# eth-ait/GauSTAR

Measured on AMD Instinct MI355X. Metric: views/sec fwd+bwd @1920x1080, 500k Gaussians; HBM GB/s vs roofline, higher is better.
Workload: dtype f32

## Files before the change

gaustar_amd/csrc/gsr_api.hip:

```cpp
#include "../../include/gsr.h"
#include "gsr_entry.h"
#include "gsr_internal.h"
#include "gsr_plan.h"
#include <algorithm>
#include <cmath>
#include <cstdio>
#include <cstdlib>
#include <cstring>
#include <string>
#include <vector>
#include <atomic>
#include <chrono>
#include <map>
#include <mutex>
#include <utility>

using namespace gsr;

namespace gsr { uint64_t* g_trace = nullptr; }

namespace {
thread_local std::string g_err;
thread_local uint32_t g_pinned_seq = 0;
thread_local uint32_t* g_pinned = nullptr;
// ... 657 lines not shown
int gsr_backward(int P, int D, int M, int R, int num_segments, const float* background, int W, int H,
                 const float* means3D, const float* shs, const float* colors_precomp, const float* scales,
                 float scale_modifier, const float* rotations, const float* cov3D_precomp, const float* viewmatrix,
                 const float* projmatrix, const float* campos, float tan_fovx, float tan_fovy, const int* radii,
                 const void* geom_buffer, const void* binning_buffer, const void* image_buffer, const float* dL_dpix,
                 void* grad_scratch, float* dL_dmean2D, float* dL_dopacity, float* dL_dcolor, float* dL_dmean3D,
                 float* dL_dcov3D, float* dL_dsh, float* dL_dscale, float* dL_drot, gsr_stream_t stream)
{
    return gsr_backward_mt(P, D, M, R, num_segments, 3, background, W, H, means3D, shs, colors_precomp, scales,
                           scale_modifier, rotations, cov3D_precomp, viewmatrix, projmatrix, campos, tan_fovx, tan_fovy,
                           radii, geom_buffer, binning_buffer, image_buffer, dL_dpix, grad_scratch, dL_dmean2D,
                           dL_dopacity, dL_dcolor, dL_dmean3D, dL_dcov3D, dL_dsh, dL_dscale, dL_drot, 0, stream);
}

int gsr_backward_mt(int P, int D, int M, int R, int num_segments, int num_channels, const float* background, int W,
                    int H, const float* means3D,
                 const float* shs, const float* colors_precomp, const float* scales, float scale_modifier,
                 const float* rotations, const float* cov3D_precomp, const float* viewmatrix, const float* projmatrix,
                 const float* campos, float tan_fovx, float tan_fovy, const int* radii, const void* geom_buffer,
                 const void* binning_buffer, const void* image_buffer, const float* dL_dpix, void* grad_scratch,
                 float* dL_dmean2D, float* dL_dopacity, float* dL_dcolor, float* dL_dmean3D, float* dL_dcov3D,
                 float* dL_dsh, float* dL_dscale, float* dL_drot, int grad_scratch_zeroed, gsr_stream_t stream)
{
    g_err.clear();
    if (P <= 0) return 0;
    if (W <= 0 || H <= 0) return fail_msg("gsr_backward: image size must be positive");
    if (!means3D || !viewmatrix || !projmatrix || !campos || !radii || !geom_buffer || !image_buffer || !dL_dpix ||
        !background)
        return fail_msg("gsr_backward: required pointer is null");
    if (!grad_scratch || !dL_dmean2D || !dL_dopacity || !dL_dcolor || !dL_dmean3D || (cov3D_precomp && !dL_dcov3D))
        return fail_msg("gsr_backward: required gradient pointer is null");
    if (shs && !dL_dsh) return fail_msg("gsr_backward: dL_dsh is null in SH mode");
    if (!cov3D_precomp && (!scales || !rotations || !dL_dscale || !dL_drot))
        return fail_msg("gsr_backward: scales/rotations and their gradients are required without cov3D_precomp");
    if (R > 0 && !binning_buffer) return fail_msg("gsr_backward: binning_buffer is null");
    if (R > 0 && num_segments <= 0)
        return fail_msg("gsr_backward: num_segments of the forward is required (a forward-only render cannot be differentiated)");
    if (!channels_ok(num_channels)) return fail_msg("gsr_backward: num_channels must be 3, 4 or 6");
    if (num_channels != 3 && !colors_precomp)
        return fail_msg("gsr_backward: multi-target renders need precomputed colours [P, num_channels]");
    const int C = num_channels;
    hipStream_t st = (hipStream_t)stream;
    ImageState im = carve_image(const_cast<void*>(image_buffer), W, H);
    GeomState g = carve_geom(const_cast<void*>(geom_buffer), P);
    BinState b = carve_bin(const_cast<void*>(binning_buffer), nonneg(R), nonneg(num_segments), C);
    float* grad_acc = static_cast<float*>(grad_scratch);
    if (!grad_scratch_zeroed) {
        Scope sc(ST_ZERO_FILL, st);
        GSR_CHECK(hipMemsetAsync(grad_acc, 0, gsr_grad_scratch_bytes(P), st));
    }
    if (R > 0) {
        {
            Scope sc(ST_BLEND_BWD, st);
            launch_blend_bwd(C, W, H, num_segments, background, features_of(colors_precomp, g), g, im, b, dL_dpix, grad_acc, env_on("GSR_BWD_LIVE"), st);
        }
        GSR_CHECK_LAUNCH("blend_bwd_kernel");
    }
    {
        Scope sc(ST_GEOM_BWD, st);
        const ViewArgs v = view_args(P, D, M, means3D, shs, colors_precomp, nullptr, cov3D_precomp ? nullptr : scales, scale_modifier,
                                     cov3D_precomp ? nullptr : rotations, cov3D_precomp, viewmatrix, projmatrix, campos, W, H,
                                     tan_fovx, tan_fovy, const_cast<int*>(radii));
        launch_geom_bwd(v, g, C, grad_acc, dL_dmean2D, dL_dopacity, dL_dcolor, dL_dmean3D, dL_dcov3D, shs ? dL_dsh : nullptr,
                        cov3D_precomp ? nullptr : dL_dscale, cov3D_precomp ? nullptr : dL_drot, st);
    }
    GSR_CHECK_LAUNCH("geom_bwd_kernel");
    return 0;
}

int gsr_mark_visible(int P, const float* means3D, const float* viewmatrix, const float* projmatrix, uint8_t* present,
                     gsr_stream_t stream)
{
    (void)projmatrix;
    g_err.clear();
    if (P <= 0) return 0;
    if (!means3D || !viewmatrix || !present) return fail_msg("gsr_mark_visible: required pointer is null");
    launch_mark_visible(P, means3D, viewmatrix, present, (hipStream_t)stream);
    GSR_CHECK_LAUNCH("mark_visible_kernel");
    return 0;
}

int gsr_release_stream_state(gsr_stream_t stream)
{
    g_err.clear();
    hipStream_t st = (hipStream_t)stream;
    int dev = 0;
    GSR_CHECK(hipGetDevice(&dev));
    std::lock_guard<std::mutex> lk(g_cnt_mu);
    auto it = g_cnt.find(std::make_pair(dev, st));
    if (it == g_cnt.end()) return 0;
    if (it->second.busy.exchange(true)) return fail_msg("gsr_release_stream_state: a forward on this stream is in flight");
    if (it->second.base) { GSR_CHECK(hipStreamSynchronize(st)); GSR_CHECK(hipFree(it->second.base)); }
    g_cnt.erase(it);
    return 0;
}

namespace {
__global__ void __launch_bounds__(64) camera_key_kernel(const float* __restrict__ m, long long s0, long long s1, uint32_t* __restrict__ pad,
                                                        uint32_t seq)
{
    const int lane = threadIdx.x;
    if (lane < 16) pad[lane] = __float_as_uint(m[(long long)(lane >> 2) * s0 + (long long)(lane & 3) * s1]);
    __threadfence_system();
    if (lane == 0) __hip_atomic_store(&pad[16], seq, __ATOMIC_RELEASE, __HIP_MEMORY_SCOPE_SYSTEM);
}
std::mutex g_key_mu;
std::map<int, hipStream_t> g_key_stream;
// ... 188 lines not shown
```

gaustar_amd/csrc/gsr_blend_bwd.hip:

```cpp
#include "gsr_bwd_util.h"

namespace gsr {

#ifndef GSR_QUAD_WAVES
#define GSR_QUAD_WAVES 7
#endif
#ifndef GSR_QUAD_WAVES4
#define GSR_QUAD_WAVES4 7
#endif
#ifndef GSR_QUAD_WAVES6
#define GSR_QUAD_WAVES6 5
#endif
#ifndef GSR_QUAD_EXP
#define GSR_QUAD_EXP 0
#endif

#ifndef GSR_QUAD_Q
#define GSR_QUAD_Q 32
#endif
#ifndef GSR_QUAD_Q6
#define GSR_QUAD_Q6 32
#endif
template <int C> struct QuadLds {
    static constexpr int Q = C == 6 ? GSR_QUAD_Q6 : GSR_QUAD_Q;
    static_assert(Q == 16 || Q == 32, "whole trips");
    static constexpr int REC_B = C <= 4 ? 48 : 64;
    static constexpr int MOM_B = C <= 4 ? 48 : 64;
    static constexpr int STG_B = C <= 4 ? 32 : 48;
    static constexpr int REC = 0;
    static constexpr int MOM = REC + (Q + 1) * REC_B;
    static constexpr int STG = MOM + (Q + 1) * MOM_B;
    static constexpr int LST = STG + 64 * STG_B;
    static constexpr int ORW = LST + 4 * Q + 16;
    static constexpr int TOTAL = ORW + 32;
    static_assert(STG % 16 == 0 && MOM % 16 == 0 && LST % 16 == 0 && ORW % 16 == 0, "16-byte accesses");
    static_assert((REC_B / 16) * Q < 256 && 6 + C + 2 <= MOM_B / 4, "list bytes; two pad words per moment record");
};

typedef uint32_t u32x2q __attribute__((ext_vector_type(2)));

__device__ __forceinline__ float fold32(float a, float b)
{
    const u32x2q r = __builtin_amdgcn_permlane32_swap(__float_as_uint(a), __float_as_uint(b), false, false);
    return __uint_as_float(r[0]) + __uint_as_float(r[1]);
}
__device__ __forceinline__ float fold16(float a, float b)
{
    const u32x2q r = __builtin_amdgcn_permlane16_swap(__float_as_uint(a), __float_as_uint(b), false, false);
    return __uint_as_float(r[0]) + __uint_as_float(r[1]);
}
__device__ __forceinline__ float fold_quad(float v)
{
    float t = v + __uint_as_float((uint32_t)__builtin_amdgcn_update_dpp(0, (int)__float_as_uint(v), 0xB1, 0xf, 0xf, true));
    return t + __uint_as_float((uint32_t)__builtin_amdgcn_update_dpp(0, (int)__float_as_uint(t), 0x4E, 0xf, 0xf, true));
}

template <int C>
__global__ void __launch_bounds__(64) __attribute__((amdgpu_waves_per_eu(C == 6 ? GSR_QUAD_WAVES6 : C == 4 ? GSR_QUAD_WAVES4 : GSR_QUAD_WAVES, 8)))
blend_bwd_kernel(int W, int H, int gx, const uint4* __restrict__ unit_info, const float4* __restrict__ snap,
                      const uint2* __restrict__ masks, const uint32_t* __restrict__ point_list, const float4* __restrict__ rec_a,
                      const float4* __restrict__ rec_b, const RecTail<C>* __restrict__ rec_c, const float* __restrict__ bg,
                      const float* __restrict__ final_T, const uint32_t* __restrict__ n_contrib,
                      const float* __restrict__ dL_dpix, float* __restrict__ grad_acc, uint64_t* __restrict__ trace,
                      const uint32_t* __restrict__ order, uint32_t live_off)
{
    using L = QuadLds<C>;
    const uint64_t t_start = trace ? wall_clock64() : 0;
    constexpr int Q = L::Q, REC_B = L::REC_B, MOM_B = L::MOM_B, STG_B = L::STG_B, REC = L::REC, MOM = L::MOM, STG = L::STG, LST = L::LST,
                  ORW = L::ORW, TOTAL = L::TOTAL, RV = REC_B / 16;
    static_assert(C == 3 || C == 4 || C == 6, "channel counts of the C ABI");
    constexpr int SV = snap_vecs(C), NM = 6 + C;
    __shared__ __attribute__((aligned(16))) unsigned char lds[TOTAL];
    const uint32_t n_units = gridDim.x >> 2;
    const uint32_t xcd = blockIdx.x & 7u, slot_id = blockIdx.x >> 3;
    const uint32_t grp = slot_id >> 2;
    uint32_t unit = (grp >> 3) * 64u + xcd * 8u + (grp & 7u);
    uint32_t wave_sel = slot_id & 3u;
    const uint32_t full = (n_units >> 6) << 6;
    if (blockIdx.x >= full * 4u) { unit = blockIdx.x >> 2; wave_sel = blockIdx.x & 3u; }
    if (order != nullptr) unit = order[unit];
    const uint4 info = unit_info[unit];
    const uint32_t live4 = (info.x >> UNIT_LIVE_SHIFT) | live_off;
    const int tile = (int)(info.x & UNIT_TILE_MASK);
    const uint32_t list0 = info.y;
    const int n = (int)info.z;
    const uint32_t unit0 = info.w;
    const int s0 = (int)(unit - unit0) * 64;
    if ((s0 >= n) | (((live4 >> wave_sel) & 1u) == 0u)) return;
    const int wave = (int)wave_sel, lane = threadIdx.x;
    const int tx = tile % gx, ty = tile / gx;
    const int sx = tx * TILE + (wave & 1) * SUB, sy = ty * TILE + (wave >> 1) * SUB;
    const int px = sx + (lane & 7), py = sy + (lane >> 3);
    const bool inside = px < W && py < H;
    const int s1 = min(s0 + BSEG, n);
    const bool has_next = s1 < n;
    const uint32_t pix = (uint32_t)W * (uint32_t)py + (uint32_t)px;
    const uint32_t HW = (uint32_t)H * (uint32_t)W;
    const auto at32 = [](const auto* base, uint32_t byte_off) {
        return *reinterpret_cast<std::remove_reference_t<decltype(*base)>*>(reinterpret_cast<const char*>(base) + byte_off);
    };
    float T_final = 0.f;
    int my_last = 0;
    float dp[C];
#pragma unroll
    for (int ch = 0; ch < C; ch++) dp[ch] = 0.f;
    if (inside) {
        T_final = at32(final_T, pix * 4u);
        my_last = (int)at32(n_contrib, pix * 4u);
#pragma unroll
        for (int ch = 0; ch < C; ch++) dp[ch] = at32(dL_dpix, ((uint32_t)ch * HW + pix) * 4u);
    }
    const uint2* const my_words = masks + ((size_t)unit * 4 + wave) * 64 + (uint32_t)lane;
    const uint2* const words_u = masks + ((size_t)unit * 4 + wave) * 64;
    uint2 word = at32(words_u, (uint32_t)lane * 8u);
    uint2 word_next = at32(words_u + (has_next ? 256 : 0), (uint32_t)lane * 8u);
    const int pidx = 16 * (py - ty * TILE) + (px - tx * TILE);
    float Ts, Tf, cs[C], cf[C];
// ... 38 lines not shown
            const uint32_t u_end = unit0 + (uint32_t)(n + 63) / 64u;
            const auto words_of = [&](uint32_t u) { const uint2 w_ = my_words[(size_t)(u - unit) * 256]; return w_.x | w_.y; };
            do { useg++; } while (useg + 1u < u_end && words_of(useg) == 0u);
            load_snapshot<C>(snap + ((size_t)useg * 256 + pidx) * SV, Ts, cs);
        }
        const float inv = __builtin_amdgcn_rcpf(Ts);
        T = Ts;
#pragma unroll
        for (int ch = 0; ch < C; ch++) acc[ch] = (cf[ch] - cs[ch]) * inv;
    }
    float accd = 0.f;
#pragma unroll
    for (int ch = 0; ch < C; ch++) accd = __builtin_fmaf(acc[ch], dp[ch], accd);
    {
        const int lim = my_lim - s0;
        word.x &= lim >= 32 ? 0xffffffffu : lim > 0 ? (1u << lim) - 1u : 0u;
        word.y &= lim >= 64 ? 0xffffffffu : lim > 32 ? (1u << (lim - 32)) - 1u : 0u;
    }
    const uint32_t lds0 = lds_byte_address(lds);
    unsigned long long ks[4];
    {
        const uint32_t sub = (uint32_t)(((lane >> 5) << 1) | ((lane >> 2) & 1));
        const uint32_t ad = lds0 + ORW + 8u * sub;
        const u32x2q zero = {0u, 0u}, mine = {word.x, word.y};
        u32x4 a01, a23;
        asm volatile("ds_write_b64 %2, %3\n\t"
                     "ds_or_b64 %2, %4\n\t"
                     "ds_read_b128 %0, %5\n\t"
                     "ds_read_b128 %1, %5 offset:16\n\t"
                     "s_waitcnt lgkmcnt(0)"
                     : "=&v"(a01), "=&v"(a23) : "v"(ad), "v"(zero), "v"(mine), "v"(lds0 + ORW) : "memory");
        const auto rfl = [](uint32_t v) { return (uint32_t)__builtin_amdgcn_readfirstlane((int)v); };
        ks[0] = ((unsigned long long)rfl(a01[1]) << 32) | rfl(a01[0]);
        ks[1] = ((unsigned long long)rfl(a01[3]) << 32) | rfl(a01[2]);
        ks[2] = ((unsigned long long)rfl(a23[1]) << 32) | rfl(a23[0]);
        ks[3] = ((unsigned long long)rfl(a23[3]) << 32) | rfl(a23[2]);
    }
    const unsigned long long kany = ks[0] | ks[1] | ks[2] | ks[3];
    if (kany == 0ull) return;
    {
        float4* st = reinterpret_cast<float4*>(lds + STG + STG_B * lane);
        st[0] = make_float4(T, accd, __uint_as_float((uint32_t)my_lim), tf_bg);
        st[1] = make_float4(dp[0], dp[1], dp[2], C > 3 ? dp[3 < C ? 3 : 0] : 0.f);
        if constexpr (C == 6) st[2] = make_float4(dp[4 < C ? 4 : 0], dp[5 < C ? 5 : 0], 0.f, 0.f);
    }
    const bool keep = ((kany >> (63 - lane)) & 1ull) != 0ull;
    const unsigned long long m = __ballot(keep);
    const int cnt_all = __popcll(m);
    float4 ra_ = ra, rb_ = rb;
    float rcc[4];
#pragma unroll
    for (int i = 0; i < 4; i++) rcc[i] = i < C - 2 ? rc.c[i < C - 2 ? i : 0] : 0.f;
    uint32_t gid_ = gid;
    for (int q0 = 0; q0 < (GSR_QUAD_EXP == 2 ? 0 : cnt_all); q0 += Q) {
        const int cnt = min(cnt_all - q0, Q);
        const int slot = (int)__builtin_amdgcn_mbcnt_hi((uint32_t)(m >> 32), __builtin_amdgcn_mbcnt_lo((uint32_t)m, 0u)) - q0;
        const bool mine = ((m >> lane) & 1ull) != 0ull && slot >= 0 && slot < Q;
        if (q0 > 0) {
            const uint32_t kl2 = (uint32_t)(min(s0 + 63 - lane, n - 1) - s0);
            ra_ = at32(rec_a + list0 + s0, kl2 * 16u);
            rb_ = at32(rec_b + list0 + s0, kl2 * 16u);
            const RecTail<C> rc2 = at32(rec_c + list0 + s0, kl2 * (uint32_t)sizeof(RecTail<C>));
#pragma unroll
            for (int i = 0; i < C - 2; i++) rcc[i] = rc2.c[i];
            gid_ = at32(point_list + list0 + s0, kl2 * 4u);
        }
        if (mine) {
            float4* r = reinterpret_cast<float4*>(lds + REC + slot * REC_B);
            r[0] = make_float4(ra_.x, ra_.y, ra_.z, ra_.w);
            r[1] = make_float4(rb_.x, rb_.y, __uint_as_float((uint32_t)(s0 + 63 - lane)), __uint_as_float(gid_));
            r[2] = make_float4(rb_.z, rb_.w, rcc[0], rcc[1]);
            if constexpr (C == 6) r[3] = make_float4(rcc[2], rcc[3], 0.f, 0.f);
        }
        if (lane == 0) {
            float4* r = reinterpret_cast<float4*>(lds + REC + Q * REC_B);
            r[0] = make_float4(0.f, 0.f, 0.f, 0.f);
            r[1] = make_float4(0.f, 0.f, __uint_as_float(0x7fffffffu), 0.f);
            r[2] = make_float4(0.f, 0.f, 0.f, 0.f);
            if constexpr (C == 6) r[3] = make_float4(0.f, 0.f, 0.f, 0.f);
        }
        for (int i = lane; i < (Q + 1) * (MOM_B / 16); i += 64) reinterpret_cast<float4*>(lds + MOM)[i] = make_float4(0.f, 0.f, 0.f, 0.f);
        if (lane < Q + 4) reinterpret_cast<uint32_t*>(lds + LST)[lane] = 0x01010101u * (uint32_t)(RV * Q);
        __builtin_amdgcn_wave_barrier();
        int cnt_s[4];
#pragma unroll
        for (int s = 0; s < 4; s++) {
            const bool in_s = mine && ((ks[s] >> (63 - lane)) & 1ull) != 0ull;
            const unsigned long long ms = __ballot(in_s);
            cnt_s[s] = __popcll(ms);
            if (in_s) {
                const int rank = (int)__builtin_amdgcn_mbcnt_hi((uint32_t)(ms >> 32), __builtin_amdgcn_mbcnt_lo((uint32_t)ms, 0u));
                lds[LST + s * Q + (rank & 3) * (Q / 4) + (rank >> 2)] = (unsigned char)(RV * slot);
            }
        }
        __builtin_amdgcn_wave_barrier();
#pragma unroll 1
        for (int s = 0; s < (GSR_QUAD_EXP ? 0 : 4); s++) {
            const int ns = s == 0 ? cnt_s[0] : s == 1 ? cnt_s[1] : s == 2 ? cnt_s[2] : cnt_s[3];
            if (ns == 0) continue;
            int lane_o = lane;
            if constexpr (C == 4) asm volatile("" : "+v"(lane_o));
            const int rho = lane_o >> 4, jj = (lane_o >> 2) & 3, kap = lane_o & 3;
            const int mom_idx = kap == 0 ? ((rho & 1) * 2 + (rho >> 1))
                              : kap == 1 ? 4 + ((rho & 1) * 2 + (rho >> 1))
                              : (kap == 2 && C == 6) ? 8 + ((rho & 1) * 2 + (rho >> 1))
                              : (kap == 2 && rho == 0) ? 8
                              : (kap == 2 && rho == 2 && C == 4) ? 9
                                                                 : NM + (lane_o & 1);
            const int bx = s & 1, by = s >> 1;
            const int pl = 8 * (4 * by + rho) + 4 * bx + kap;
            const float4* st = reinterpret_cast<const float4*>(lds + STG + STG_B * pl);
            const float4 s_a = st[0], s_b = st[1];
            float d4 = 0.f, d5 = 0.f;
            if constexpr (C == 6) { const float4 s_c = st[2]; d4 = s_c.x; d5 = s_c.y; }
            float Tp = s_a.x, Ap = s_a.y;
            const int lim = (int)__float_as_uint(s_a.z);
            const float tfbg = s_a.w;
            const float d0 = s_b.x, d1 = s_b.y, d2 = s_b.z, d3 = s_b.w;
            const float pxf = (float)(sx + 4 * bx + kap), pyf = (float)(sy + 4 * by + rho);
            const int ntrip = (ns + 3) >> 2;
            SlotRegs<RV> rec;
            const uint32_t lst_ad = lds0 + LST + (uint32_t)(s * Q + jj * (Q / 4));
            uint32_t idx_nxt;
            asm volatile("ds_read_u8 %0, %1\n\ts_waitcnt lgkmcnt(0)" : "=v"(idx_nxt) : "v"(lst_ad) : "memory");
            uint32_t ad = (idx_nxt << 4) + (lds0 + REC);
            lds_request<RV, 0>(rec, ad);
            asm volatile("ds_read_u8 %0, %1 offset:1" : "=v"(idx_nxt) : "v"(lst_ad) : "memory");
#pragma unroll 1
            for (int t = 0; t < ntrip; t++) {
                lds_wait<0>(rec);
                asm volatile("" : "+v"(idx_nxt));
                const uint32_t mom_ad = ad + (uint32_t)(MOM - REC) + 4u * (uint32_t)mom_idx;
                float mom_old;
                asm volatile("ds_read_b32 %0, %1" : "=v"(mom_old) : "v"(mom_ad) : "memory");
// ... 20 lines not shown
                asm volatile("s_nop 1\n\t"
                             "v_mul_f32_dpp %0, %4, %0 row_ror:4 row_mask:0xf bank_mask:0x1\n\t"
                             "v_fmac_f32_dpp %2, %5, %1 row_ror:4 row_mask:0xf bank_mask:0x1\n\t"
                             "s_nop 0\n\t"
                             "v_mul_f32_dpp %0, %0, %0 row_shr:4 row_mask:0xf bank_mask:0xf\n\t"
                             "v_fmac_f32_dpp %2, %2, %1 row_shr:4 row_mask:0xf bank_mask:0xf\n\t"
                             "v_mul_f32_dpp %1, %1, %1 row_shr:4 row_mask:0xf bank_mask:0xf\n\t"
                             "v_mul_f32_dpp %0, %0, %0 row_shr:8 row_mask:0xf bank_mask:0xf\n\t"
                             "s_nop 0\n\t"
                             "v_fmac_f32_dpp %2, %2, %1 row_shr:8 row_mask:0xf bank_mask:0xf\n\t"
                             "v_subrev_f32_dpp %3, %5, %6 row_ror:4 row_mask:0xf bank_mask:0xf\n\t"
                             "s_nop 0\n\t"
                             "v_subrev_f32_dpp %3, %2, %6 row_shr:4 row_mask:0xf bank_mask:0xf"
                             : "+v"(x), "+v"(A), "+v"(B), "=&v"(sdl) : "v"(Tp), "v"(Ap), "v"(kd));
                Tp = x;
                Ap = B;
                const float w = ae * x;
                const float u = __builtin_fmaf(sdl, x, -(rinv * tfbg));
                const float r = live ? G * u : 0.0f;
                typedef float f32x2p __attribute__((ext_vector_type(2)));
                const f32x2p dxy = {dx, dy}, d01 = {d0, d1};
                const f32x2p p12 = r * dxy;
                const f32x2p p34 = p12[0] * dxy;
                const float p5 = p12[1] * dy;
                const f32x2p p67 = w * d01;
                const float p8 = w * d2;
                float p8b = C > 3 ? w * d3 : p8;
                if constexpr (C == 3) asm volatile("" : "+v"(p8b));
                const float f01 = fold32(r, p12[0]), f23 = fold32(p12[1], p34[0]), f45 = fold32(p34[1], p5), f67 = fold32(p67[0], p67[1]),
                            f88 = fold32(p8, p8b);
                float f88b = f88;
                if constexpr (C == 6) f88b = fold32(w * d4, w * d5);
                else asm volatile("" : "+v"(f88b));
                const float gA = fold16(f01, f23);
                const float gB = fold16(f45, f67);
                const float gC = fold16(f88, f88b);
                const float hA = fold_quad(gA), hB = fold_quad(gB), hC = fold_quad(gC);
                const float val = kap == 0 ? hA : kap == 1 ? hB : hC;
                if constexpr (RV == 3) asm volatile("s_waitcnt lgkmcnt(4)" : "+v"(mom_old) : : "memory");
                else asm volatile("s_waitcnt lgkmcnt(5)" : "+v"(mom_old) : : "memory");
                const float mom_new = mom_old + val;
                asm volatile("ds_write_b32 %0, %1" : : "v"(mom_ad), "v"(mom_new) : "memory");
            }
            lds_wait<0>(rec);
            asm volatile("" : "+v"(idx_nxt));
            if (jj == 3) {
                float2* stw = reinterpret_cast<float2*>(lds + STG + STG_B * pl);
                *stw = make_float2(Tp, Ap);
            }
            __builtin_amdgcn_wave_barrier();
        }
        asm volatile("s_waitcnt lgkmcnt(0)" : : : "memory");
        __builtin_amdgcn_wave_barrier();
        for (int idx = lane; idx < cnt * NM; idx += 64) {
            const int e = idx / NM, v = idx - e * NM;
            const size_t g = __float_as_uint(reinterpret_cast<const float*>(lds + REC + e * REC_B)[7]);
            atomic_add_f32(grad_acc + g * GRAD_RS + v, reinterpret_cast<const float*>(lds + MOM + e * MOM_B)[v]);
        }
        __builtin_amdgcn_wave_barrier();
    }
    if (trace && lane == 0) {
        if (wave == 0) trace[2 * unit] = t_start;
        atomicMax((unsigned long long*)&trace[2 * unit + 1], (unsigned long long)wall_clock64());
    }
}

#ifdef GSR_BWD_VARIANT
bool launch_blend_bwd_variant(int C, int W, int H, int U, const float* bg, ImageState im, BinState b, const float* dL_dpix, float* grad_acc,
                              hipStream_t st);
#endif
const uint32_t* g_bwd_order = nullptr;

void launch_blend_bwd(int C, int W, int H, int U, const float* bg, const float* feats, GeomState g, ImageState im,
                      BinState b, const float* dL_dpix, float* grad_acc, bool use_live, hipStream_t st)
{
    (void)feats; (void)g;
    if (U <= 0) return;
    const uint32_t live_off = use_live ? 0u : 0xfu;
#ifdef GSR_BWD_VARIANT
    if (launch_blend_bwd_variant(C, W, H, U, bg, im, b, dL_dpix, grad_acc, st)) return;
#endif
    static const int pad = getenv("GSR_BWD_LDS_PAD") ? atoi(getenv("GSR_BWD_LDS_PAD")) : 0;
    const Tiles t = tiles_of(W, H);
    uint64_t* tr = g_trace ? g_trace + 2 * (size_t)t.T : nullptr;
    if (C == 3)
        blend_bwd_kernel<3><<<4 * U, 64, pad, st>>>(W, H, t.gx, b.unit_info, b.snap, b.masks, b.point_list, b.rec_a, b.rec_b,
                                                    static_cast<const RecTail<3>*>(b.rec_c), bg, im.final_T, im.n_contrib, dL_dpix, grad_acc, tr, g_bwd_order, live_off);
    else if (C == 4)
        blend_bwd_kernel<4><<<4 * U, 64, pad, st>>>(W, H, t.gx, b.unit_info, b.snap, b.masks, b.point_list, b.rec_a, b.rec_b,
                                                    static_cast<const RecTail<4>*>(b.rec_c), bg, im.final_T, im.n_contrib, dL_dpix, grad_acc, tr, g_bwd_order, live_off);
    else
        blend_bwd_kernel<6><<<4 * U, 64, pad, st>>>(W, H, t.gx, b.unit_info, b.snap, b.masks, b.point_list, b.rec_a, b.rec_b,
                                                    static_cast<const RecTail<6>*>(b.rec_c), bg, im.final_T, im.n_contrib, dL_dpix, grad_acc, tr, g_bwd_order, live_off);
}

}
```

gaustar_amd/csrc/gsr_blend_fwd.hip:

```cpp
#include "gsr_internal.h"
#include "gsr_mask.h"
#include "gsr_sort.h"
#include "gsr_plan.h"
#include <cstdlib>

namespace gsr {

#ifndef GSR_FWD_LIGHT_TILES
#define GSR_FWD_LIGHT_TILES 16
#endif
constexpr int FWD_LIGHT_TILES = GSR_FWD_LIGHT_TILES;
static_assert(FWD_LIGHT_TILES >= 1 && FWD_LIGHT_TILES <= 64, "a wave's lanes hold the group's tiles");

template <int C, int CH, int MODE, bool PLANNED = false>
__global__ void __launch_bounds__(256)
blend_fwd_kernel(int W, int H, int gx, const uint2* __restrict__ ranges, const uint32_t* __restrict__ order,
                 uint32_t* point_list, const uint64_t* __restrict__ sort_keys, const float4* __restrict__ g0,
                 const float4* __restrict__ g1,
                 const float* __restrict__ feats, const float* __restrict__ bg, float* __restrict__ out_color,
                 float* __restrict__ final_T, uint32_t* __restrict__ n_contrib, const uint32_t* __restrict__ seg_off,
                 uint2* __restrict__ masks, uint4* __restrict__ unit_info, float4* __restrict__ snap, float4* __restrict__ rec_a, float4* __restrict__ rec_b,
                 RecTail<C>* __restrict__ rec_c, const uint2* __restrict__ part_list, const uint32_t* __restrict__ totals,
                 float4* __restrict__ part_fin, uint32_t* __restrict__ part_last, uint32_t* __restrict__ part_ticket,
                 uint32_t part_grid, bool parts_sort, uint32_t split_n, bool keep,
// ... 158 lines not shown
#endif
#ifndef GSR_FWD_SORT_STAGGER
#define GSR_FWD_SORT_STAGGER 1
#endif
#ifndef GSR_FWD_TAIL_PRIO
#define GSR_FWD_TAIL_PRIO 704
#endif
    const auto prio_by_length = [&]() {
        if (GSR_FWD_TAIL_PRIO && tile_block >= (uint32_t)GSR_FWD_TAIL_PRIO && n > 0u) { __builtin_amdgcn_s_setprio(3); return; }
        if (n > 1024u) __builtin_amdgcn_s_setprio(3);
        else if (n > 704u) __builtin_amdgcn_s_setprio(2);
        else if (n > 448u) __builtin_amdgcn_s_setprio(1);
    };
#if GSR_FWD_SORT_STAGGER
    if (GSR_FWD_TAIL_PRIO && tile_block >= (uint32_t)GSR_FWD_TAIL_PRIO && n > 0u) __builtin_amdgcn_s_setprio(3);
    else switch ((tile_block >> 8) & 3u) {
        case 0: __builtin_amdgcn_s_setprio(3); break;
        case 1: __builtin_amdgcn_s_setprio(2); break;
        case 2: __builtin_amdgcn_s_setprio(1); break;
        default: __builtin_amdgcn_s_setprio(0); break;
    }
#else
    prio_by_length();
#endif
    const uint64_t* ids_lds = nullptr;
    if (!is_part) {
        if (sort_keys != nullptr) {
#ifdef GSR_FWD_PHASES
            if (n >= 1u && n <= 2048u) ids_lds = sort_small_tile(reinterpret_cast<uint64_t*>(smem), sort_keys + list0, point_list + list0, n, [&]() { FWD_PHASE(); });
#else
            if (n >= 1u && n <= 2048u) ids_lds = sort_small_tile(reinterpret_cast<uint64_t*>(smem), sort_keys + list0, point_list + list0, n);
#endif
            __syncthreads();
            FWD_PHASE();
        }
#if GSR_FWD_SORT_STAGGER
        prio_by_length();
#endif
    } else if (parts_sort && sort_keys != nullptr && n <= SORT_SMALL_CAP) {
        sort_small_tile(reinterpret_cast<uint64_t*>(smem), sort_keys + list0, point_list + list0, n);
        __syncthreads();
    }
    const uint32_t* list = point_list + list0;
    const TransposeConsts tc(lane);

    float T = 1.0f;
    float Cc[C];
#pragma unroll
    for (int ch = 0; ch < C; ch++) Cc[ch] = 0.f;
    uint32_t last = 0;
    uint32_t live = 0;
    bool done = !inside;
    uint32_t seg_cur = (is_part && part_c0 != 0u) ? 0xffffffffu : 0u;

    uint32_t gid_nxt[PT];
    float4 a_nxt[PT], b_nxt[PT];
    float col_nxt[PT][C];
    const auto fetch_ids = [&](uint32_t c0) {
#pragma unroll
        for (int q = 0; q < PT; q++) {
            const uint32_t k = c0 + q * 256 + threadIdx.x;
            gid_nxt[q] = k < n ? (ids_lds != nullptr ? (uint32_t)ids_lds[k] : list[k]) : 0xffffffffu;
        }
    };
    const auto fetch_records = [&]() {
#pragma unroll
        for (int q = 0; q < PT; q++) {
            const uint32_t gid = gid_nxt[q];
            a_nxt[q] = make_float4(0.f, 0.f, 1.f, 0.f);
            b_nxt[q] = make_float4(1.f, 0.f, -1.f, 0.f);
#pragma unroll
            for (int ch = 0; ch < C; ch++) col_nxt[q][ch] = 0.f;
            if (gid != 0xffffffffu) {
                a_nxt[q] = g0[gid];
                b_nxt[q] = g1[gid];
                if constexpr (C % 2 == 0) {
                    const float2* pf = reinterpret_cast<const float2*>(feats + (size_t)C * gid);
#pragma unroll
                    for (int ch = 0; ch < C; ch += 2) { const float2 v = pf[ch / 2]; col_nxt[q][ch] = v.x; col_nxt[q][ch + 1] = v.y; }
                } else {
#pragma unroll
                    for (int ch = 0; ch < C; ch++) col_nxt[q][ch] = feats[(size_t)C * gid + ch];
                }
            }
        }
    };
    const auto park = [&](uint32_t c0, bool words_known, bool words_out, bool recs_out) {
        const uint32_t u_lo = c0 >> 6;
#pragma unroll
        for (int q = 0; q < PT; q++) {
            const InstRec<C> rec = make_rec<C>(a_nxt[q], b_nxt[q], col_nxt[q]);
            ga[q * 256 + threadIdx.x] = rec.a;
            gb[q * 256 + threadIdx.x] = rec.b;
            gc[q * 256 + threadIdx.x] = rec.t;
            if (recs_out) {
                const uint32_t k = c0 + q * 256 + threadIdx.x;
                if (k < n) {
                    rec_a[list0 + k] = rec.a;
                    rec_b[list0 + k] = rec.b;
                    rec_c[list0 + k] = rec.t;
                }
            }
            if (c0 + q * 256 + wave * 64 < n) {
                const int hw = 2 * (4 * q + wave);
                uint2* const gm = masks + ((size_t)(unit0 + u_lo + 4 * q + wave) * 4) * 64 + lane;
                if (words_known) {
// ... 5 lines not shown
                    }
                } else {
                    unit_masks(a_nxt[q], b_nxt[q], tx * TILE, ty * TILE, tc, [&](int blk, uint32_t lo, uint32_t hi) {
                        mk[blk][hw][lane] = lo;
                        mk[blk][hw + 1][lane] = hi;
                        if (words_out) gm[blk * 64] = make_uint2(lo, hi);
                    });
                }
            }
        }
    };
    const auto nonempty_words = [&](uint32_t c0) {
        uint32_t nz = 0;
#pragma unroll
        for (int hh = 0; hh < NH; hh++)
            if (c0 + 32u * hh < n) nz |= (mk[wave][hh][lane] != 0u ? 1u : 0u) << hh;
        return nz;
    };
#ifndef GSR_FWD_PIPE
#define GSR_FWD_PIPE 1
#endif
#if GSR_FWD_PIPE
    typedef float f32x4_ __attribute__((ext_vector_type(4)));
    typedef float f32x2_ __attribute__((ext_vector_type(2)));
    using TailRegs = std::conditional_t<sizeof(RecTail<C>) == 4, float, std::conditional_t<sizeof(RecTail<C>) == 8, f32x2_, f32x4_>>;
    struct RecRegs { f32x4_ a, b; TailRegs k; };
    const uint32_t ga_addr = (uint32_t)(size_t)ga, gc_addr = (uint32_t)(size_t)gc;
    const auto request = [&](RecRegs& r, uint32_t slot) {
        const uint32_t ad = ga_addr + slot * 16u;
        asm volatile("ds_read_b128 %0, %1" : "=&v"(r.a) : "v"(ad) : "memory");
        asm volatile("ds_read_b128 %0, %1 offset:%2" : "=&v"(r.b) : "v"(ad), "n"(16 * CH) : "memory");
        const uint32_t ak = gc_addr + slot * (uint32_t)sizeof(RecTail<C>);
        if constexpr (sizeof(RecTail<C>) == 4) asm volatile("ds_read_b32 %0, %1" : "=&v"(r.k) : "v"(ak) : "memory");
        else if constexpr (sizeof(RecTail<C>) == 8) asm volatile("ds_read_b64 %0, %1" : "=&v"(r.k) : "v"(ak) : "memory");
        else asm volatile("ds_read_b128 %0, %1" : "=&v"(r.k) : "v"(ak) : "memory");
    };
    const auto walk = [&](uint32_t c0, uint32_t nz) {
        const uint32_t mk_lane = (uint32_t)(size_t)&mk[wave][0][lane];
        uint32_t cur = 0, nw = 0;
        int h = 0, nh = 0;
        bool stopped = false;
        if (nz != 0u) { h = __builtin_ctz(nz); cur = mk[wave][h][lane]; nz &= nz - 1u; }
        if (nz != 0u) { nh = __builtin_ctz(nz); nw = mk[wave][nh][lane]; nz &= nz - 1u; }
        uint32_t slot = (uint32_t)(h * 32 + __builtin_ctz(cur | 0x80000000u));
        RecRegs rec0, rec1;
        request(rec0, slot);
        asm volatile("s_waitcnt lgkmcnt(0)" : "+v"(rec0.a), "+v"(rec0.b), "+v"(rec0.k) : : "memory");
        const auto trip = [&](RecRegs& rec, RecRegs& nxt) {
            const bool act = cur != 0u;
            if (snaps || is_part) {
                const uint32_t seg_new = (c0 + (uint32_t)h * 32u) / (uint32_t)SNAP_SEG;
                if (act && seg_new != seg_cur) {
                    seg_cur = seg_new;
                    store_snapshot<C>(snap + ((size_t)(unit0 + seg_new * (SNAP_SEG / 64)) * 256 + pix_in_tile) * SV, T, Cc);
                }
            }
            const uint32_t rest = cur & (cur - 1u);
            const bool exhausted = rest == 0u;
            const uint32_t ncur = exhausted ? nw : rest;
            const int nh2 = exhausted ? nh : h;
            const uint32_t nslot = (uint32_t)(nh2 * 32 + __builtin_ctz(ncur | 0x80000000u));
            const int t = __builtin_ctz(nz | 0x80000000u) & (NH - 1);
            uint32_t wnext;
            asm volatile("ds_read_b32 %0, %1" : "=v"(wnext) : "v"(mk_lane + (uint32_t)t * 256u) : "memory");
            request(nxt, nslot);
            asm volatile("" : "+v"(rec.a), "+v"(rec.b), "+v"(rec.k));
            float col[C];
            col[0] = rec.b[2]; col[1] = rec.b[3];
            if constexpr (C == 3) col[2] = rec.k;
            else {
#pragma unroll
                for (int ch = 2; ch < C; ch++) col[ch] = rec.k[ch - 2];
            }
            const float dx = rec.a[0] - pxf, dy = rec.a[1] - pyf;
            const float power = pair_exp2_arg(rec.a[2], rec.a[3], rec.b[0], dx, dy);
            const float alpha = fminf(ALPHA_MAX, rec.b[1] * __builtin_amdgcn_exp2f(power));
            const bool ok = act && power <= 0.0f && alpha >= ALPHA_MIN;
            const float test_T = T * (1.0f - alpha);
            const bool stop = ok && test_T < T_EPS;
            const bool upd = ok != stop;
            const float w = upd ? alpha * T : 0.0f;
#pragma unroll
            for (int ch = 0; ch < C; ch++) Cc[ch] += col[ch] * w;
            T = upd ? test_T : T;
            last = upd ? c0 + slot + 1u : last;
            live |= (upd ? 1u : 0u) << (((c0 + slot) >> 6) & 31u);
            if constexpr (C == 3)
                asm volatile("s_waitcnt lgkmcnt(0)" : "+v"(wnext), "+v"(nxt.a), "+v"(nxt.b), "+v"(nxt.k), "+v"(T), "+v"(last), "+v"(Cc[0]), "+v"(Cc[1]), "+v"(Cc[2]) : : "memory");
            else if constexpr (C == 4)
                asm volatile("s_waitcnt lgkmcnt(0)" : "+v"(wnext), "+v"(nxt.a), "+v"(nxt.b), "+v"(nxt.k), "+v"(T), "+v"(last), "+v"(Cc[0]), "+v"(Cc[1]), "+v"(Cc[2]), "+v"(Cc[3]) : : "memory");
            else
                asm volatile("s_waitcnt lgkmcnt(0)" : "+v"(wnext), "+v"(nxt.a), "+v"(nxt.b), "+v"(nxt.k), "+v"(T), "+v"(last), "+v"(Cc[0]), "+v"(Cc[1]), "+v"(Cc[2]), "+v"(Cc[3]), "+v"(Cc[4]), "+v"(Cc[5]) : : "memory");
            cur = ncur;
            h = nh2;
            nw = exhausted ? (nz != 0u ? wnext : 0u) : nw;
            nh = exhausted ? t : nh;
            nz = exhausted ? (nz & (nz - 1u)) : nz;
            stopped = stopped || stop;
            cur = stop ? 0u : cur;
            nw = stop ? 0u : nw;
            nz = stop ? 0u : nz;
            slot = nslot;
        };
        while (__ballot(cur != 0u) != 0ull) {
            trip(rec0, rec1);
            trip(rec1, rec0);
        }
// ... 363 lines not shown
```

gaustar_amd/csrc/gsr_internal.h:

```cpp
#pragma once
#include <cstdlib>
#include <hip/hip_runtime.h>
#include <stdint.h>
#include <stddef.h>

namespace gsr {

constexpr int TILE = 16;
constexpr int SUB = 8;
constexpr float NEAR_Z = 0.2f;
constexpr float ALPHA_MIN = 1.0f / 255.0f;
constexpr float ALPHA_MAX = 0.99f;
constexpr float T_EPS = 0.0001f;

struct Tiles { int gx, gy, T; };
__host__ __device__ inline Tiles tiles_of(int W, int H)
{
    Tiles t; t.gx = (W + TILE - 1) / TILE; t.gy = (H + TILE - 1) / TILE; t.T = t.gx * t.gy; return t;
}

__host__ __device__ inline size_t align_up(size_t x) { return (x + 255) & ~(size_t)255; }

struct GeomState {
    float4* g0;
// ... 191 lines not shown
    uint32_t n_light;
};

extern uint64_t* g_trace;
extern const uint32_t* g_bwd_order;

struct Camera {
    float view[16];
    float proj[16];
    float campos[3];
    float tan_fovx, tan_fovy, focal_x, focal_y;
    int W, H;
};

struct ViewArgs {
    int P, D, M;
    const float* means3D;
    const float* shs;
    const float* colors_precomp;
    const float* opacities;
    const float* scales;
    float scale_modifier;
    const float* rotations;
    const float* cov3D_precomp;
    const float* viewmatrix;
    const float* projmatrix;
    const float* campos;
    int W, H;
    float tan_fovx, tan_fovy;
    int* radii;
    Tiles tiles() const { return tiles_of(W, H); }
};

void launch_preprocess(const ViewArgs& v, GeomState g, ImageState im, uint32_t view_token, hipStream_t st);
void launch_preprocess_planned(const ViewArgs& v, GeomState g, ImageState im, PlanRun plan, hipStream_t st);
void launch_tile_scan(ImageState im, int T, uint32_t* host_totals, uint32_t host_seq, uint32_t view_token, hipStream_t st);
void launch_scatter(int P, int W, int H, int R, uint32_t max_count, GeomState g, ImageState im, BinState b, hipStream_t st);
void launch_scatter_early(int P, int W, int H, int C, GeomState g, ImageState im, void* binning_base, size_t capacity, hipStream_t st);
bool launch_tile_sort(int W, int H, int R, int U, uint32_t max_count, ImageState im, BinState b, bool blend_sorts_small, hipStream_t st);
bool tile_sort_launches(int R, uint32_t max_count, bool blend_sorts_small);
inline int front_of_order(int R, int T)
{
    const long long bound = ((long long)(R > 0 ? R : 0) / 2017 + 1 + 255) / 256 * 256;
    return (int)(bound < (long long)T ? bound : (long long)T);
}
struct PlanJob;
void launch_blend_fwd_planned(int C, int W, int H, const float* bg, const float* feats, GeomState g, ImageState im, BinState b,
                              float* out_color, bool keep_masks, void* zero_ptr, size_t zero_bytes, PlanRun plan, hipStream_t st,
                              const PlanJob* job = nullptr);
void launch_blend_fwd(int C, int W, int H, int R, int U, uint32_t max_count, const float* bg, const float* feats, GeomState g, ImageState im,
                      BinState b, float* out_color, bool keep_masks, void* zero_ptr, size_t zero_bytes, uint32_t* counters,
                      bool sort_small, hipStream_t st, const PlanJob* job = nullptr, bool* job_rides = nullptr, int num_parts = -1);
void launch_blend_bwd(int C, int W, int H, int U, const float* bg, const float* feats, GeomState g, ImageState im, BinState b,
                      const float* dL_dpix, float* grad_acc, bool use_live, hipStream_t st);
void launch_geom_bwd(const ViewArgs& v, GeomState g, int C, const float* grad_acc, float* dL_dmean2D, float* dL_dopacity,
                     float* dL_dcolor, float* dL_dmean3D, float* dL_dcov3D, float* dL_dsh, float* dL_dscale, float* dL_drot,
                     hipStream_t st);
void launch_mark_visible(int P, const float* means3D, const float* view, uint8_t* present, hipStream_t st);
void preprocess_occupancy(int* exact, int* planned);

#ifdef __HIPCC__
__device__ constexpr float kSH0 = 0.28209479177387814f;
__device__ constexpr float kSH1 = 0.4886025119029199f;
__device__ constexpr float kSH2[5] = {1.0925484305920792f, -1.0925484305920792f, 0.31539156525252005f,
                                      -1.0925484305920792f, 0.5462742152960396f};
__device__ constexpr float kSH3[7] = {-0.5900435899266435f, 2.890611442640554f, -0.4570457994644658f,
                                      0.3731763325901154f, -0.4570457994644658f, 1.445305721320277f,
                                      -0.5900435899266435f};
__device__ constexpr float kSH4[9] = {2.5033429417967046f, -1.7701307697799304f, 0.9461746957575601f,
                                      -0.6690465435572892f, 0.10578554691520431f, -0.6690465435572892f,
                                      0.47308734787878004f, -1.7701307697799304f, 0.6258357354491761f};
constexpr int SH_MAX_BASIS = 25;

struct Vec3 { float x, y, z; };

__device__ __forceinline__ Vec3 load3(const float* p, size_t i) { return Vec3{p[3 * i], p[3 * i + 1], p[3 * i + 2]}; }

__device__ __forceinline__ Vec3 xform43(const Vec3 p, const float* m)
{
    return Vec3{m[0] * p.x + m[4] * p.y + m[8] * p.z + m[12], m[1] * p.x + m[5] * p.y + m[9] * p.z + m[13],
                m[2] * p.x + m[6] * p.y + m[10] * p.z + m[14]};
}
__device__ __forceinline__ float xform4w(const Vec3 p, const float* m)
{
    return m[3] * p.x + m[7] * p.y + m[11] * p.z + m[15];
}

__device__ __forceinline__ float view_depth(const Vec3 p, const float* m)
{
#pragma clang fp contract(off)
    const float yz = m[6] * p.y;
    const float zz = m[10] * p.z;
    return (__builtin_fmaf(m[2], p.x, yz) + zz) + m[14];
}

__device__ __forceinline__ void quat_R(const float4 q, float R[3][3])
{
    const float r = q.x, x = q.y, y = q.z, z = q.w;
    R[0][0] = 1.f - 2.f * (y * y + z * z); R[0][1] = 2.f * (x * y - r * z); R[0][2] = 2.f * (x * z + r * y);
    R[1][0] = 2.f * (x * y + r * z); R[1][1] = 1.f - 2.f * (x * x + z * z); R[1][2] = 2.f * (y * z - r * x);
    R[2][0] = 2.f * (x * z - r * y); R[2][1] = 2.f * (y * z + r * x); R[2][2] = 1.f - 2.f * (x * x + y * y);
}

__device__ __forceinline__ void cov3d_from_scale_rot(const Vec3 s_in, float mod, const float4 q, float c[6])
{
    float R[3][3];
    quat_R(q, R);
// ... 393 lines not shown
```

gaustar_amd/csrc/gsr_sort.h:

```cpp
#pragma once
#include "gsr_internal.h"

namespace gsr {

template <int D>
__device__ __forceinline__ uint32_t lane_xor_u32(uint32_t v)
{
    if constexpr (D == 1) return (uint32_t)__builtin_amdgcn_mov_dpp((int)v, 0xB1, 0xf, 0xf, true);
    else if constexpr (D == 2) return (uint32_t)__builtin_amdgcn_mov_dpp((int)v, 0x4E, 0xf, 0xf, true);
    else if constexpr (D == 4) return (uint32_t)__builtin_amdgcn_ds_swizzle((int)v, 0x101F);
    else if constexpr (D == 8) return (uint32_t)__builtin_amdgcn_ds_swizzle((int)v, 0x201F);
    else if constexpr (D == 16) return (uint32_t)__builtin_amdgcn_ds_swizzle((int)v, 0x401F);
    else return (uint32_t)__shfl_xor((int)v, 32, 64);
}
template <int E, int D>
__device__ __forceinline__ void cross_lane_stage(uint64_t (&v)[E], uint32_t e0, uint32_t k, int lane)
{
    const bool lower = (lane & D) == 0;
#pragma unroll
    for (int r = 0; r < E; r++) {
        const uint64_t pv = ((uint64_t)lane_xor_u32<D>((uint32_t)(v[r] >> 32)) << 32) | lane_xor_u32<D>((uint32_t)v[r]);
        const bool asc = ((e0 + r) & k) == 0;
        const bool take_min = lower == asc;
        const bool gt = v[r] > pv;
// ... 117 lines not shown
#define GSR_SORT_KARY 4
#endif
#if GSR_SORT_KARY == 4
            while (lo < hi) {
                const uint32_t span = hi - lo;
                const uint32_t m1 = lo + (span >> 2), m2 = lo + (span >> 1), m3 = lo + ((3u * span) >> 2);
                const uint64_t a1 = a[m1], b1 = b[d - 1u - m1], a2 = a[m2], b2 = b[d - 1u - m2], a3 = a[m3], b3 = b[d - 1u - m3];
                const bool p1 = a1 < b1, p2 = a2 < b2, p3 = a3 < b3;
                if (!p1) hi = m1;
                else if (!p2) { lo = m1 + 1u; hi = m2; }
                else if (!p3) { lo = m2 + 1u; hi = m3; }
                else lo = m3 + 1u;
            }
#else
            while (lo < hi) {
                const uint32_t mid = (lo + hi) >> 1;
                if (a[mid] < b[d - 1u - mid]) lo = mid + 1u; else hi = mid;
            }
#endif
            const uint32_t ai = lo, bi = d - lo;
            uint64_t ka[E], kb[E];
#pragma unroll
            for (int e = 0; e < E; e++) {
                ka[e] = ai + (uint32_t)e < la ? a[ai + e] : ~0ull;
                kb[e] = bi + (uint32_t)e < lb ? b[bi + e] : ~0ull;
            }
#pragma unroll
            for (int e = 0; e < E; e++) res[e] = ka[e] < kb[E - 1 - e] ? ka[e] : kb[E - 1 - e];
#pragma unroll
            for (int j = E / 2; j > 0; j >>= 1) {
#pragma unroll
                for (int e = 0; e < E; e++) {
                    if ((e & j) == 0) {
                        const uint64_t x = res[e], y = res[e | j];
                        const bool gt = x > y;
                        res[e] = gt ? y : x;
                        res[e | j] = gt ? x : y;
                    }
                }
            }
#pragma unroll
            for (int e = 0; e < E; e++)
                if (o0 + (uint32_t)e < n) B[o0 + e] = res[e];
        }
        __syncthreads();
        stamp();
        uint64_t* t = A; A = B; B = t;
    }
    if (out_keys != nullptr) { for (uint32_t i = tid; i < n; i += 256u) out_keys[i] = A[i]; }
    else { for (uint32_t i = tid; i < n; i += 256u) out[i] = (uint32_t)A[i]; }
    return A;
}

template <class STAMP = NoStamp>
__device__ __forceinline__ const uint64_t* sort_small_tile(uint64_t* __restrict__ s, const uint64_t* __restrict__ gk,
                                                           uint32_t* __restrict__ out, uint32_t n, STAMP stamp = STAMP())
{
    if (n == 1) {
        if (threadIdx.x == 0) out[0] = (uint32_t)gk[0];
        return nullptr;
    }
    if (n <= 512u) return sort_tile_merge<2>(s, gk, out, n, nullptr, stamp);
    if (n <= 1024u) return sort_tile_merge<4>(s, gk, out, n, nullptr, stamp);
    return sort_tile_merge<8>(s, gk, out, n, nullptr, stamp);
}

}
```

Baseline: 5316.

## Cheapen blend-backward flush addressing, hoist sentinel, trim LDS zeroing, 32-bit snapshot offsets

The backward blend flush now uses a multiply-shift in place of integer division and stores a precomputed byte offset (gid times row stride) in the record, so the atomic address is a 32-bit add unless the gradient buffer exceeds 4 GiB. The sentinel record write moves out of the per-batch loop, and moment zeroing covers only cnt records instead of Q+1. The forward snapshot store uses 32-bit byte offsets when the list is small enough. The sort tile selection is also rewritten around configurable E macros whose defaults give the same behaviour. These changes cut integer ALU and LDS work in hot loops, at the cost of added specialised paths and one more kernel argument.

After: 5304. About the same (-0.2%).

```diff
diff --git a/gaustar_amd/csrc/gsr_api.hip b/gaustar_amd/csrc/gsr_api.hip
--- a/gaustar_amd/csrc/gsr_api.hip
+++ b/gaustar_amd/csrc/gsr_api.hip
@@ -733,7 +733,7 @@
     if (R > 0) {
         {
             Scope sc(ST_BLEND_BWD, st);
-            launch_blend_bwd(C, W, H, num_segments, background, features_of(colors_precomp, g), g, im, b, dL_dpix, grad_acc, env_on("GSR_BWD_LIVE"), st);
+            launch_blend_bwd(C, W, H, num_segments, background, features_of(colors_precomp, g), g, im, b, dL_dpix, grad_acc, P, env_on("GSR_BWD_LIVE"), st);
         }
         GSR_CHECK_LAUNCH("blend_bwd_kernel");
     }
diff --git a/gaustar_amd/csrc/gsr_blend_bwd.hip b/gaustar_amd/csrc/gsr_blend_bwd.hip
--- a/gaustar_amd/csrc/gsr_blend_bwd.hip
+++ b/gaustar_amd/csrc/gsr_blend_bwd.hip
@@ -37,6 +37,17 @@
     static_assert((REC_B / 16) * Q < 256 && 6 + C + 2 <= MOM_B / 4, "list bytes; two pad words per moment record");
 };
 
+template <int NM> struct FlushDiv {
+    static_assert(NM == 9 || NM == 10 || NM == 12, "6 + C moments");
+    static constexpr uint32_t MUL = NM == 9 ? 57u : NM == 10 ? 205u : 171u, SHIFT = NM == 9 ? 9u : 11u;
+    static constexpr bool exact_below(uint32_t n)
+    {
+        for (uint32_t i = 0; i < n; i++)
+            if (((i * MUL) >> SHIFT) != i / (uint32_t)NM) return false;
+        return true;
+    }
+};
+
 typedef uint32_t u32x2q __attribute__((ext_vector_type(2)));
 
 __device__ __forceinline__ float fold32(float a, float b)
@@ -62,7 +73,7 @@
                       const float4* __restrict__ rec_b, const RecTail<C>* __restrict__ rec_c, const float* __restrict__ bg,
                       const float* __restrict__ final_T, const uint32_t* __restrict__ n_contrib,
                       const float* __restrict__ dL_dpix, float* __restrict__ grad_acc, uint64_t* __restrict__ trace,
-                      const uint32_t* __restrict__ order, uint32_t live_off)
+                      const uint32_t* __restrict__ order, uint32_t live_off, uint32_t wide_acc)
 {
     using L = QuadLds<C>;
     const uint64_t t_start = trace ? wall_clock64() : 0;
@@ -207,6 +218,14 @@
 #pragma unroll
     for (int i = 0; i < 4; i++) rcc[i] = i < C - 2 ? rc.c[i < C - 2 ? i : 0] : 0.f;
     uint32_t gid_ = gid;
+    if (lane == 0) {
+        float4* r = reinterpret_cast<float4*>(lds + REC + Q * REC_B);
+        r[0] = make_float4(0.f, 0.f, 0.f, 0.f);
+        r[1] = make_float4(0.f, 0.f, __uint_as_float(0x7fffffffu), 0.f);
+        r[2] = make_float4(0.f, 0.f, 0.f, 0.f);
+        if constexpr (C == 6) r[3] = make_float4(0.f, 0.f, 0.f, 0.f);
+    }
+    const uint32_t row_scale = wide_acc ? 1u : (uint32_t)(GRAD_RS * sizeof(float));
     for (int q0 = 0; q0 < (GSR_QUAD_EXP == 2 ? 0 : cnt_all); q0 += Q) {
         const int cnt = min(cnt_all - q0, Q);
         const int slot = (int)__builtin_amdgcn_mbcnt_hi((uint32_t)(m >> 32), __builtin_amdgcn_mbcnt_lo((uint32_t)m, 0u)) - q0;
@@ -223,18 +242,11 @@
         if (mine) {
             float4* r = reinterpret_cast<float4*>(lds + REC + slot * REC_B);
             r[0] = make_float4(ra_.x, ra_.y, ra_.z, ra_.w);
-            r[1] = make_float4(rb_.x, rb_.y, __uint_as_float((uint32_t)(s0 + 63 - lane)), __uint_as_float(gid_));
+            r[1] = make_float4(rb_.x, rb_.y, __uint_as_float((uint32_t)(s0 + 63 - lane)), __uint_as_float(gid_ * row_scale));
             r[2] = make_float4(rb_.z, rb_.w, rcc[0], rcc[1]);
             if constexpr (C == 6) r[3] = make_float4(rcc[2], rcc[3], 0.f, 0.f);
         }
-        if (lane == 0) {
-            float4* r = reinterpret_cast<float4*>(lds + REC + Q * REC_B);
-            r[0] = make_float4(0.f, 0.f, 0.f, 0.f);
-            r[1] = make_float4(0.f, 0.f, __uint_as_float(0x7fffffffu), 0.f);
-            r[2] = make_float4(0.f, 0.f, 0.f, 0.f);
-            if constexpr (C == 6) r[3] = make_float4(0.f, 0.f, 0.f, 0.f);
-        }
-        for (int i = lane; i < (Q + 1) * (MOM_B / 16); i += 64) reinterpret_cast<float4*>(lds + MOM)[i] = make_float4(0.f, 0.f, 0.f, 0.f);
+        for (int i = lane; i < cnt * (MOM_B / 16); i += 64) reinterpret_cast<float4*>(lds + MOM)[i] = make_float4(0.f, 0.f, 0.f, 0.f);
         if (lane < Q + 4) reinterpret_cast<uint32_t*>(lds + LST)[lane] = 0x01010101u * (uint32_t)(RV * Q);
         __builtin_amdgcn_wave_barrier();
         int cnt_s[4];
@@ -361,10 +373,25 @@
         }
         asm volatile("s_waitcnt lgkmcnt(0)" : : : "memory");
         __builtin_amdgcn_wave_barrier();
-        for (int idx = lane; idx < cnt * NM; idx += 64) {
-            const int e = idx / NM, v = idx - e * NM;
-            const size_t g = __float_as_uint(reinterpret_cast<const float*>(lds + REC + e * REC_B)[7]);
-            atomic_add_f32(grad_acc + g * GRAD_RS + v, reinterpret_cast<const float*>(lds + MOM + e * MOM_B)[v]);
+        {
+            static_assert(REC_B == MOM_B, "one byte offset for an instance's record and its moments");
+            static_assert(FlushDiv<NM>::exact_below(Q * NM) && 4u * Q * NM * FlushDiv<NM>::MUL < (1u << 24), "the flush's division");
+            const uint32_t end4 = (uint32_t)(cnt * NM) * 4u;
+            const auto flush = [&](auto wide) {
+                for (uint32_t i4 = (uint32_t)lane * 4u; i4 < end4; i4 += 256u) {
+                    const uint32_t e = __umul24(i4, FlushDiv<NM>::MUL) >> (FlushDiv<NM>::SHIFT + 2);
+                    const uint32_t eo = __umul24(e, (uint32_t)MOM_B);
+                    const uint32_t v4 = i4 - __umul24(e, 4u * NM);
+                    const uint32_t row = *reinterpret_cast<const uint32_t*>(lds + REC + 28 + eo);
+                    const float sum = *reinterpret_cast<const float*>(lds + MOM + (i4 + __umul24(e, (uint32_t)(MOM_B - 4 * NM))));
+                    if constexpr (!decltype(wide)::value)
+                        atomic_add_f32(reinterpret_cast<float*>(reinterpret_cast<char*>(grad_acc) + (row + v4)), sum);
+                    else
+                        atomic_add_f32(grad_acc + (size_t)row * GRAD_RS + (v4 >> 2), sum);
+                }
+            };
+            if (!wide_acc) flush(std::false_type());
+            else flush(std::true_type());
         }
         __builtin_amdgcn_wave_barrier();
     }
@@ -381,11 +408,12 @@
 const uint32_t* g_bwd_order = nullptr;
 
 void launch_blend_bwd(int C, int W, int H, int U, const float* bg, const float* feats, GeomState g, ImageState im,
-                      BinState b, const float* dL_dpix, float* grad_acc, bool use_live, hipStream_t st)
+                      BinState b, const float* dL_dpix, float* grad_acc, int P, bool use_live, hipStream_t st)
 {
     (void)feats; (void)g;
     if (U <= 0) return;
     const uint32_t live_off = use_live ? 0u : 0xfu;
+    const uint32_t wide = (uint64_t)P * GRAD_RS * sizeof(float) > 0xffffffffull ? 1u : 0u;
 #ifdef GSR_BWD_VARIANT
     if (launch_blend_bwd_variant(C, W, H, U, bg, im, b, dL_dpix, grad_acc, st)) return;
 #endif
@@ -394,13 +422,13 @@
     uint64_t* tr = g_trace ? g_trace + 2 * (size_t)t.T : nullptr;
     if (C == 3)
         blend_bwd_kernel<3><<<4 * U, 64, pad, st>>>(W, H, t.gx, b.unit_info, b.snap, b.masks, b.point_list, b.rec_a, b.rec_b,
-                                                    static_cast<const RecTail<3>*>(b.rec_c), bg, im.final_T, im.n_contrib, dL_dpix, grad_acc, tr, g_bwd_order, live_off);
+                                                    static_cast<const RecTail<3>*>(b.rec_c), bg, im.final_T, im.n_contrib, dL_dpix, grad_acc, tr, g_bwd_order, live_off, wide);
     else if (C == 4)
         blend_bwd_kernel<4><<<4 * U, 64, pad, st>>>(W, H, t.gx, b.unit_info, b.snap, b.masks, b.point_list, b.rec_a, b.rec_b,
-                                                    static_cast<const RecTail<4>*>(b.rec_c), bg, im.final_T, im.n_contrib, dL_dpix, grad_acc, tr, g_bwd_order, live_off);
+                                                    static_cast<const RecTail<4>*>(b.rec_c), bg, im.final_T, im.n_contrib, dL_dpix, grad_acc, tr, g_bwd_order, live_off, wide);
     else
         blend_bwd_kernel<6><<<4 * U, 64, pad, st>>>(W, H, t.gx, b.unit_info, b.snap, b.masks, b.point_list, b.rec_a, b.rec_b,
-                                                    static_cast<const RecTail<6>*>(b.rec_c), bg, im.final_T, im.n_contrib, dL_dpix, grad_acc, tr, g_bwd_order, live_off);
-}
-
-}
+                                                    static_cast<const RecTail<6>*>(b.rec_c), bg, im.final_T, im.n_contrib, dL_dpix, grad_acc, tr, g_bwd_order, live_off, wide);
+}
+
+}
diff --git a/gaustar_amd/csrc/gsr_blend_fwd.hip b/gaustar_amd/csrc/gsr_blend_fwd.hip
--- a/gaustar_amd/csrc/gsr_blend_fwd.hip
+++ b/gaustar_amd/csrc/gsr_blend_fwd.hip
@@ -234,6 +234,13 @@
     uint32_t live = 0;
     bool done = !inside;
     uint32_t seg_cur = (is_part && part_c0 != 0u) ? 0xffffffffu : 0u;
+#ifndef GSR_FWD_SNAP32
+#define GSR_FWD_SNAP32 1
+#endif
+    constexpr uint32_t SNAP_SEG_PIX = (uint32_t)(SNAP_SEG / 64) * 256u;
+    constexpr uint32_t SNAP32_MAX_N = GSR_FWD_SNAP32 ? 1u << 24 : 0u;
+    static_assert((uint64_t)(SNAP32_MAX_N / 64u + 1u) * 256u * SV * 16u < (1ull << 32), "32-bit snapshot offsets");
+    char* const snap_tile = reinterpret_cast<char*>(snap + (size_t)unit0 * 256 * SV);
 
     uint32_t gid_nxt[PT];
     float4 a_nxt[PT], b_nxt[PT];
@@ -345,7 +352,9 @@
                 const uint32_t seg_new = (c0 + (uint32_t)h * 32u) / (uint32_t)SNAP_SEG;
                 if (act && seg_new != seg_cur) {
                     seg_cur = seg_new;
-                    store_snapshot<C>(snap + ((size_t)(unit0 + seg_new * (SNAP_SEG / 64)) * 256 + pix_in_tile) * SV, T, Cc);
+                    const uint32_t sp = seg_new * SNAP_SEG_PIX + (uint32_t)pix_in_tile;
+                    if (n <= SNAP32_MAX_N) store_snapshot<C>(reinterpret_cast<float4*>(snap_tile + sp * ((uint32_t)SV * 16u)), T, Cc);
+                    else store_snapshot<C>(reinterpret_cast<float4*>(snap_tile) + (size_t)sp * SV, T, Cc);
                 }
             }
             const uint32_t rest = cur & (cur - 1u);
diff --git a/gaustar_amd/csrc/gsr_internal.h b/gaustar_amd/csrc/gsr_internal.h
--- a/gaustar_amd/csrc/gsr_internal.h
+++ b/gaustar_amd/csrc/gsr_internal.h
@@ -267,7 +267,7 @@
                       BinState b, float* out_color, bool keep_masks, void* zero_ptr, size_t zero_bytes, uint32_t* counters,
                       bool sort_small, hipStream_t st, const PlanJob* job = nullptr, bool* job_rides = nullptr, int num_parts = -1);
 void launch_blend_bwd(int C, int W, int H, int U, const float* bg, const float* feats, GeomState g, ImageState im, BinState b,
-                      const float* dL_dpix, float* grad_acc, bool use_live, hipStream_t st);
+                      const float* dL_dpix, float* grad_acc, int P, bool use_live, hipStream_t st);
 void launch_geom_bwd(const ViewArgs& v, GeomState g, int C, const float* grad_acc, float* dL_dmean2D, float* dL_dopacity,
                      float* dL_dcolor, float* dL_dmean3D, float* dL_dcov3D, float* dL_dsh, float* dL_dscale, float* dL_drot,
                      hipStream_t st);
diff --git a/gaustar_amd/csrc/gsr_sort.h b/gaustar_amd/csrc/gsr_sort.h
--- a/gaustar_amd/csrc/gsr_sort.h
+++ b/gaustar_amd/csrc/gsr_sort.h
@@ -193,6 +193,15 @@
     return A;
 }
 
+#ifndef GSR_SORT_E_256
+#define GSR_SORT_E_256 2
+#endif
+#ifndef GSR_SORT_E_512
+#define GSR_SORT_E_512 2
+#endif
+#ifndef GSR_SORT_E_1024
+#define GSR_SORT_E_1024 4
+#endif
 template <class STAMP = NoStamp>
 __device__ __forceinline__ const uint64_t* sort_small_tile(uint64_t* __restrict__ s, const uint64_t* __restrict__ gk,
                                                            uint32_t* __restrict__ out, uint32_t n, STAMP stamp = STAMP())
@@ -201,8 +210,11 @@
         if (threadIdx.x == 0) out[0] = (uint32_t)gk[0];
         return nullptr;
     }
-    if (n <= 512u) return sort_tile_merge<2>(s, gk, out, n, nullptr, stamp);
-    if (n <= 1024u) return sort_tile_merge<4>(s, gk, out, n, nullptr, stamp);
+    constexpr int E256 = GSR_SORT_E_256, E512 = GSR_SORT_E_512, E1024 = GSR_SORT_E_1024;
+    static_assert(E256 >= 1 && E512 >= 2 && E1024 >= 4 && E256 <= 8 && E512 <= 8 && E1024 <= 8, "256 E keys hold the list");
+    if (E256 != E512 && n <= 256u) return sort_tile_merge<E256>(s, gk, out, n, nullptr, stamp);
+    if (E512 != E1024 && n <= 512u) return sort_tile_merge<E512>(s, gk, out, n, nullptr, stamp);
+    if (E1024 != 8 && n <= 1024u) return sort_tile_merge<E1024>(s, gk, out, n, nullptr, stamp);
     return sort_tile_merge<8>(s, gk, out, n, nullptr, stamp);
 }
 
```
